# delafrouzmir/test-resilient-osss-ucx

Measured on AMD Instinct MI355X. Metric: GiB/s device-resident shmem_double_sum_to_all combine + %HBM peak, 1/2/4/8 GPU, higher is better.
Workload: dtype f64; 1 GPU; BASELINE config 2: shmem_double_sum_to_all combine, nreduce=64Mi, K=2 inputs (source + peer source), 1 MI355X, device-resident combine kernel; nreduce=67108864, K=2

## Files before the change

test-resilient-osss-ucx_amd/csrc/copy.hip:

```cpp
#include <hip/hip_runtime.h>

#include <stdint.h>
#include <stdlib.h>

#include "combine.hpp"

namespace osgpu {
namespace {

typedef unsigned int u32x4 __attribute__((ext_vector_type(4)));
typedef u32x4 u32x4_a4 __attribute__((aligned(4)));

constexpr int kThreads = 256;
constexpr int kU = 4;
constexpr size_t kBlockBytes = (size_t) kThreads * kU * 16;

struct SegTable {
    const char *src[kMaxCopySegs];
    char *dst[kMaxCopySegs];
    size_t bytes[kMaxCopySegs];
    unsigned first_block[kMaxCopySegs + 1];
    unsigned rounds;
    int n;
};

__device__ __forceinline__ int find_seg(const SegTable &t, unsigned b)
{
    int k = 0;
#pragma unroll
    for (int i = 1; i < kMaxCopySegs; i++)
        if (i < t.n && b >= t.first_block[i]) k = i;
    return k;
}

__global__ __launch_bounds__(kThreads) void copy_vec_kernel(SegTable t)
{
    const unsigned inter = t.rounds * (unsigned) t.n;
    int k;
    unsigned lb;
    if (blockIdx.x < inter) {
        k = (int) (blockIdx.x % (unsigned) t.n);
        lb = blockIdx.x / (unsigned) t.n;
    } else {
        const unsigned b = blockIdx.x - inter;
        k = find_seg(t, b);
        lb = t.rounds + (b - t.first_block[k]);
    }
    const char *s = t.src[k];
    char *d = t.dst[k];
    const size_t bytes = t.bytes[k];
    size_t head = (size_t) ((0 - (uintptr_t) d) & 15);
    if (head > bytes) head = bytes;
    const size_t nvec = (bytes - head) / 16;
    const size_t tail0 = head + nvec * 16;
    if (lb == 0) {
        const unsigned x = threadIdx.x;
        if (x < head) d[x] = s[x];
        if (x < bytes - tail0) d[tail0 + x] = s[tail0 + x];
    }
    const u32x4_a4 *sv = reinterpret_cast<const u32x4_a4 *>(s + head);
    u32x4 *dv = reinterpret_cast<u32x4 *>(d + head);
    const size_t base = (size_t) lb * kThreads * kU + threadIdx.x;
    u32x4 v[kU];
#pragma unroll
    for (int u = 0; u < kU; u++) {
        const size_t i = base + (size_t) u * kThreads;
        if (i < nvec) v[u] = __builtin_nontemporal_load(sv + i);
    }
#pragma unroll
    for (int u = 0; u < kU; u++) {
        const size_t i = base + (size_t) u * kThreads;
        if (i < nvec) __builtin_nontemporal_store(v[u], dv + i);
    }
}

__global__ __launch_bounds__(kThreads) void copy_byte_kernel(SegTable t)
{
    const int k = find_seg(t, blockIdx.x);
    const size_t per_block = (size_t) kThreads * 16;
    const size_t lo = (size_t) (blockIdx.x - t.first_block[k]) * per_block;
    for (size_t i = lo + threadIdx.x; i < t.bytes[k] && i < lo + per_block; i += kThreads)
        t.dst[k][i] = t.src[k][i];
}

__global__ __launch_bounds__(kThreads) void probe_load_kernel(const unsigned long long *src,
                                                              unsigned long long *dst,
                                                              unsigned words)
{
    if (threadIdx.x < words) dst[threadIdx.x] = src[threadIdx.x];
}

__global__ __launch_bounds__(kThreads) void host_copy_kernel(const char *__restrict__ s,
                                                             char *__restrict__ d, size_t bytes)
{
    size_t head = (size_t) ((0 - (uintptr_t) d) & 15);
    if (head > bytes) head = bytes;
    const size_t nvec = (bytes - head) / 16;
    const size_t tail0 = head + nvec * 16;
    if (blockIdx.x == 0) {
        const unsigned x = threadIdx.x;
        if (x < head) d[x] = s[x];
        if (x < bytes - tail0) d[tail0 + x] = s[tail0 + x];
    }
    const u32x4_a4 *sv = reinterpret_cast<const u32x4_a4 *>(s + head);
    u32x4 *dv = reinterpret_cast<u32x4 *>(d + head);
    const size_t stride = (size_t) gridDim.x * kThreads * kU;
    for (size_t base = (size_t) blockIdx.x * kThreads * kU + threadIdx.x; base < nvec;
         base += stride) {
        u32x4 v[kU];
#pragma unroll
        for (int u = 0; u < kU; u++) {
            const size_t i = base + (size_t) u * kThreads;
            if (i < nvec) v[u] = __builtin_nontemporal_load(sv + i);
        }
#pragma unroll
        for (int u = 0; u < kU; u++) {
            const size_t i = base + (size_t) u * kThreads;
            if (i < nvec) dv[i] = v[u];
        }
    }
}

}

hipError_t launch_host_copy(void *dst, const void *src, size_t bytes, hipStream_t stream)
{
    static const unsigned grid = [] {
        const char *e = getenv("OSGPU_HOST_COPY_GRID");
        const long v = e ? atol(e) : 256;
        return (unsigned) (v < 1 ? 1 : (v > 4096 ? 4096 : v));
    }();
    if (bytes == 0) return hipSuccess;
    if (((uintptr_t) src ^ (uintptr_t) dst) & 3) {
        CopySeg g = {src, dst, bytes};
        return launch_copy(&g, 1, stream);
    }
    const size_t tiles = (bytes + kBlockBytes - 1) / kBlockBytes;
    hipLaunchKernelGGL(host_copy_kernel, dim3((unsigned) (tiles < grid ? tiles : grid)),
                       dim3(kThreads), 0, stream, static_cast<const char *>(src),
                       static_cast<char *>(dst), bytes);
    return hipGetLastError();
}

hipError_t launch_probe_load(const void *src, void *dst, size_t bytes, hipStream_t stream)
{
    static_assert(kProbeLoadBytes == (size_t) kThreads * 8, "one word per lane");
    if (bytes % 8 || bytes > kProbeLoadBytes || ((uintptr_t) src | (uintptr_t) dst) & 7)
        return hipErrorInvalidValue;
    hipLaunchKernelGGL(probe_load_kernel, dim3(1), dim3(kThreads), 0, stream,
                       static_cast<const unsigned long long *>(src),
                       static_cast<unsigned long long *>(dst), (unsigned) (bytes / 8));
    return hipGetLastError();
}

hipError_t launch_copy(const CopySeg *segs, int nseg, hipStream_t stream)
{
    SegTable vt{}, bt{};
    unsigned vblocks = 0, bblocks = 0;
    for (int i = 0; i < nseg; i++) {
        const CopySeg &g = segs[i];
        if (g.bytes == 0) continue;
        const uintptr_t phase = (uintptr_t) g.src ^ (uintptr_t) g.dst;
        SegTable &t = (phase & 3) ? bt : vt;
        unsigned &nb = (phase & 3) ? bblocks : vblocks;
        const size_t per = (phase & 3) ? (size_t) kThreads * 16 : kBlockBytes;
        const size_t blocks = (g.bytes + per - 1) / per;
        if (blocks > 0x7fffffffu - nb) return hipErrorInvalidValue;
        if (t.n == kMaxCopySegs) return hipErrorInvalidValue;
        t.src[t.n] = (const char *) g.src;
        t.dst[t.n] = (char *) g.dst;
        t.bytes[t.n] = g.bytes;
        t.first_block[t.n] = nb;
        t.n++;
        nb += (unsigned) blocks;
    }
    if (vt.n) {
        unsigned rounds = ~0u;
        for (int i = 0; i < vt.n; i++) {
            const unsigned next = i + 1 < vt.n ? vt.first_block[i + 1] : vblocks;
            rounds = next - vt.first_block[i] < rounds ? next - vt.first_block[i] : rounds;
        }
        unsigned nb = 0;
        for (int i = 0; i < vt.n; i++) {
            const unsigned next = i + 1 < vt.n ? vt.first_block[i + 1] : vblocks;
            const unsigned tiles = next - vt.first_block[i];
            vt.first_block[i] = nb;
            nb += tiles - rounds;
        }
        vt.first_block[vt.n] = nb;
        vt.rounds = rounds;
        hipLaunchKernelGGL(copy_vec_kernel, dim3(vblocks), dim3(kThreads), 0, stream, vt);
        hipError_t e = hipGetLastError();
        if (e != hipSuccess) return e;
    }
    if (bt.n) {
        bt.first_block[bt.n] = bblocks;
        hipLaunchKernelGGL(copy_byte_kernel, dim3(bblocks), dim3(kThreads), 0, stream, bt);
        hipError_t e = hipGetLastError();
        if (e != hipSuccess) return e;
    }
    return hipSuccess;
}

}
```

Measured before the change: 6246 GiB/s.

## Add wave-granular copy kernel for few-segment copies and split oversized launches

Adds a wave-sized (64-thread) copy kernel that assigns one 1KiB tile per wave, interleaving up to two segments across waves of a block, used when source and destination share 16-byte phase. Copies with more segments or mismatched phase keep the 256-thread block kernel, and both paths now split the grid into multiple launches bounded by max_launch_threads. The finer granularity aims to improve load balance and the tail of small copies, at the cost of many more tiny blocks and more scheduling overhead for large copies. The benchmarked workload is a sum_to_all combine, so this copy path may be off the timed path.

```diff
diff --git a/test-resilient-osss-ucx_amd/csrc/copy.hip b/test-resilient-osss-ucx_amd/csrc/copy.hip
--- a/test-resilient-osss-ucx_amd/csrc/copy.hip
+++ b/test-resilient-osss-ucx_amd/csrc/copy.hip
@@ -14,6 +14,9 @@
 constexpr int kThreads = 256;
 constexpr int kU = 4;
 constexpr size_t kBlockBytes = (size_t) kThreads * kU * 16;
+
+constexpr int kCopyU1 = 1, kCopyW1 = 1, kCopyUM = 1;
+constexpr int kCopyWaveMaxSegs = 2;
 
 struct SegTable {
     const char *src[kMaxCopySegs];
@@ -22,6 +25,7 @@
     unsigned first_block[kMaxCopySegs + 1];
     unsigned rounds;
     int n;
+    unsigned first;
 };
 
 __device__ __forceinline__ int find_seg(const SegTable &t, unsigned b)
@@ -36,13 +40,14 @@
 __global__ __launch_bounds__(kThreads) void copy_vec_kernel(SegTable t)
 {
     const unsigned inter = t.rounds * (unsigned) t.n;
+    const unsigned bx = t.first + blockIdx.x;
     int k;
     unsigned lb;
-    if (blockIdx.x < inter) {
-        k = (int) (blockIdx.x % (unsigned) t.n);
-        lb = blockIdx.x / (unsigned) t.n;
+    if (bx < inter) {
+        k = (int) (bx % (unsigned) t.n);
+        lb = bx / (unsigned) t.n;
     } else {
-        const unsigned b = blockIdx.x - inter;
+        const unsigned b = bx - inter;
         k = find_seg(t, b);
         lb = t.rounds + (b - t.first_block[k]);
     }
@@ -74,6 +79,55 @@
     }
 }
 
+template <int U, int W>
+__global__ __launch_bounds__(64 * W) void copy_vec_kernel_wave(SegTable t)
+{
+    constexpr size_t V = 64 * U;
+    const int w = __builtin_amdgcn_readfirstlane((int) (threadIdx.x >> 6));
+    const unsigned lane = threadIdx.x & 63;
+    const unsigned g = t.first + blockIdx.x;
+    int k;
+    size_t tile;
+    if (g < t.rounds) {
+        k = w;
+        tile = g;
+    } else {
+        const unsigned b = g - t.rounds;
+        k = find_seg(t, b);
+        tile = t.rounds + (size_t) (b - t.first_block[k]) * W + w;
+    }
+    const char *s = t.src[k];
+    char *d = t.dst[k];
+    const size_t bytes = t.bytes[k];
+    size_t head = (size_t) ((0 - (uintptr_t) d) & 15);
+    if (head > bytes) head = bytes;
+    const size_t nvec = (bytes - head) / 16;
+    const size_t tail0 = head + nvec * 16;
+    if (tile == 0) {
+        if (lane < head) d[lane] = s[lane];
+        if (lane < bytes - tail0) d[tail0 + lane] = s[tail0 + lane];
+    }
+    const size_t base = tile * V;
+    if (base >= nvec) return;
+    const u32x4_a4 *sv = reinterpret_cast<const u32x4_a4 *>(s + head) + base + lane;
+    u32x4 *dv = reinterpret_cast<u32x4 *>(d + head) + base + lane;
+    u32x4 v[U];
+    if (base + V <= nvec) {
+#pragma unroll
+        for (int u = 0; u < U; u++) v[u] = __builtin_nontemporal_load(sv + u * 64);
+#pragma unroll
+        for (int u = 0; u < U; u++) __builtin_nontemporal_store(v[u], dv + u * 64);
+    } else {
+        const size_t left = nvec - base;
+#pragma unroll
+        for (int u = 0; u < U; u++)
+            if (u * 64 + lane < left) v[u] = __builtin_nontemporal_load(sv + u * 64);
+#pragma unroll
+        for (int u = 0; u < U; u++)
+            if (u * 64 + lane < left) __builtin_nontemporal_store(v[u], dv + u * 64);
+    }
+}
+
 __global__ __launch_bounds__(kThreads) void copy_byte_kernel(SegTable t)
 {
     const int k = find_seg(t, blockIdx.x);
@@ -153,44 +207,116 @@
     return hipGetLastError();
 }
 
+template <int U, int W>
+static hipError_t launch_wave(SegTable &t, hipStream_t stream)
+{
+    constexpr size_t V = 64 * U;
+    size_t tiles[kMaxCopySegs], rounds = ~(size_t) 0;
+    for (int i = 0; i < t.n; i++) {
+        size_t head = (size_t) ((0 - (uintptr_t) t.dst[i]) & 15);
+        if (head > t.bytes[i]) head = t.bytes[i];
+        const size_t nvec = (t.bytes[i] - head) / 16;
+        tiles[i] = nvec ? (nvec + V - 1) / V : 1;
+        rounds = tiles[i] < rounds ? tiles[i] : rounds;
+    }
+    if (t.n == 1) rounds = 0;
+    size_t nb = 0;
+    for (int i = 0; i < t.n; i++) {
+        t.first_block[i] = (unsigned) nb;
+        nb += (tiles[i] - rounds + W - 1) / W;
+        if (rounds + nb > 0xffffffffu) return hipErrorInvalidValue;
+    }
+    t.first_block[t.n] = (unsigned) nb;
+    t.rounds = (unsigned) rounds;
+    const size_t groups = rounds + nb;
+    const size_t lim = max_launch_threads() / (64 * W);
+    const size_t per_launch = lim ? lim : 1;
+    for (size_t g0 = 0; g0 < groups; g0 += per_launch) {
+        const size_t ng = groups - g0 < per_launch ? groups - g0 : per_launch;
+        t.first = (unsigned) g0;
+        hipLaunchKernelGGL((copy_vec_kernel_wave<U, W>), dim3((unsigned) ng), dim3(64 * W), 0,
+                           stream, t);
+        const hipError_t e = hipGetLastError();
+        if (e != hipSuccess) return e;
+    }
+    return hipSuccess;
+}
+
+static hipError_t launch_blocks(SegTable &t, hipStream_t stream)
+{
+    size_t tiles[kMaxCopySegs], rounds = ~(size_t) 0, total = 0;
+    for (int i = 0; i < t.n; i++) {
+        tiles[i] = (t.bytes[i] + kBlockBytes - 1) / kBlockBytes;
+        rounds = tiles[i] < rounds ? tiles[i] : rounds;
+        total += tiles[i];
+        if (total > 0x7fffffffu) return hipErrorInvalidValue;
+    }
+    unsigned nb = 0;
+    for (int i = 0; i < t.n; i++) {
+        t.first_block[i] = nb;
+        nb += (unsigned) (tiles[i] - rounds);
+    }
+    t.first_block[t.n] = nb;
+    t.rounds = (unsigned) rounds;
+    const size_t lim = max_launch_threads() / kThreads;
+    const size_t per_launch = lim ? lim : 1;
+    for (size_t b0 = 0; b0 < total; b0 += per_launch) {
+        const size_t n = total - b0 < per_launch ? total - b0 : per_launch;
+        t.first = (unsigned) b0;
+        hipLaunchKernelGGL(copy_vec_kernel, dim3((unsigned) n), dim3(kThreads), 0, stream, t);
+        const hipError_t e = hipGetLastError();
+        if (e != hipSuccess) return e;
+    }
+    return hipSuccess;
+}
+
+template <int M>
+static hipError_t launch_vec(SegTable &t, hipStream_t stream)
+{
+    if constexpr (M > kCopyWaveMaxSegs)
+        return launch_blocks(t, stream);
+    else
+        return launch_wave<M == 1 ? kCopyU1 : kCopyUM, M == 1 ? kCopyW1 : M>(t, stream);
+}
+
 hipError_t launch_copy(const CopySeg *segs, int nseg, hipStream_t stream)
 {
     SegTable vt{}, bt{};
-    unsigned vblocks = 0, bblocks = 0;
+    unsigned bblocks = 0;
     for (int i = 0; i < nseg; i++) {
         const CopySeg &g = segs[i];
         if (g.bytes == 0) continue;
-        const uintptr_t phase = (uintptr_t) g.src ^ (uintptr_t) g.dst;
-        SegTable &t = (phase & 3) ? bt : vt;
-        unsigned &nb = (phase & 3) ? bblocks : vblocks;
-        const size_t per = (phase & 3) ? (size_t) kThreads * 16 : kBlockBytes;
-        const size_t blocks = (g.bytes + per - 1) / per;
-        if (blocks > 0x7fffffffu - nb) return hipErrorInvalidValue;
+        const bool bytewise = (((uintptr_t) g.src ^ (uintptr_t) g.dst) & 3) != 0;
+        SegTable &t = bytewise ? bt : vt;
         if (t.n == kMaxCopySegs) return hipErrorInvalidValue;
         t.src[t.n] = (const char *) g.src;
         t.dst[t.n] = (char *) g.dst;
         t.bytes[t.n] = g.bytes;
-        t.first_block[t.n] = nb;
+        if (bytewise) {
+            const size_t per = (size_t) kThreads * 16;
+            const size_t blocks = (g.bytes + per - 1) / per;
+            if (blocks > 0x7fffffffu - bblocks) return hipErrorInvalidValue;
+            t.first_block[t.n] = bblocks;
+            bblocks += (unsigned) blocks;
+        }
         t.n++;
-        nb += (unsigned) blocks;
     }
     if (vt.n) {
-        unsigned rounds = ~0u;
-        for (int i = 0; i < vt.n; i++) {
-            const unsigned next = i + 1 < vt.n ? vt.first_block[i + 1] : vblocks;
-            rounds = next - vt.first_block[i] < rounds ? next - vt.first_block[i] : rounds;
+        bool phased = false;
+        for (int i = 0; i < vt.n; i++)
+            phased |= (((uintptr_t) vt.src[i] ^ (uintptr_t) vt.dst[i]) & 15) != 0;
+        hipError_t e;
+        if (phased) e = launch_blocks(vt, stream);
+        else switch (vt.n) {
+        case 1: e = launch_vec<1>(vt, stream); break;
+        case 2: e = launch_vec<2>(vt, stream); break;
+        case 3: e = launch_vec<3>(vt, stream); break;
+        case 4: e = launch_vec<4>(vt, stream); break;
+        case 5: e = launch_vec<5>(vt, stream); break;
+        case 6: e = launch_vec<6>(vt, stream); break;
+        case 7: e = launch_vec<7>(vt, stream); break;
+        default: e = launch_vec<8>(vt, stream); break;
         }
-        unsigned nb = 0;
-        for (int i = 0; i < vt.n; i++) {
-            const unsigned next = i + 1 < vt.n ? vt.first_block[i + 1] : vblocks;
-            const unsigned tiles = next - vt.first_block[i];
-            vt.first_block[i] = nb;
-            nb += tiles - rounds;
-        }
-        vt.first_block[vt.n] = nb;
-        vt.rounds = rounds;
-        hipLaunchKernelGGL(copy_vec_kernel, dim3(vblocks), dim3(kThreads), 0, stream, vt);
-        hipError_t e = hipGetLastError();
         if (e != hipSuccess) return e;
     }
     if (bt.n) {
```

Result: slower. 6003 GiB/s (-3.9%).
